# juanmc2005/diart

Hardware: AMD Instinct MI355X
Metric: real-time-factor xRT streams/GPU @500ms step (higher is better)
Workload: dtype f16x3

## Files before the change

### diart_amd/_lib.py

```python
from __future__ import annotations

import ctypes as C
import os
from pathlib import Path
from typing import Optional

EXPERIMENTS = os.environ.get("DZ_EXPERIMENTS", "0") not in ("", "0")
_LIB_PATH = Path(__file__).resolve().parent / ("libdiart_amd_exp.so" if EXPERIMENTS else "libdiart_amd.so")
_lib: Optional[C.CDLL] = None

c_float_p = C.POINTER(C.c_float)
c_double_p = C.POINTER(C.c_double)
c_int_p = C.POINTER(C.c_int)
vp = C.c_void_p


class SincNetWeights(C.Structure):
    _fields_ = [("wav_gamma", C.c_float), ("wav_beta", C.c_float)] + [
        (n, vp) for n in ("filt", "in0_g", "in0_b", "w1", "b1", "in1_g", "in1_b",
                          "w2", "b2", "in2_g", "in2_b", "w1_split", "w2_split", "filt_split")]


class SegWeights(C.Structure):
    _fields_ = [("sinc", SincNetWeights), ("wih", vp * 4), ("bih", vp * 4), ("whh", vp * 4),
# ... 92 lines not shown
    "dz_resample_out_len": (C.c_longlong, [C.c_int, C.c_int, C.c_longlong]),
    "dz_resample_table": (C.c_int, [C.c_int, C.c_int, c_float_p]),
    "dz_resample_create": (C.c_int, [vp, C.c_int, C.c_int, C.POINTER(vp)]),
    "dz_resample_forward": (C.c_int, [vp, vp, C.c_longlong, C.c_longlong, C.c_int, vp, C.c_longlong, vp]),
    "dz_resample_destroy": (C.c_int, [vp]),
    "dz_prof_enable": (C.c_int, [C.c_int]),
    "dz_prof_pause": (C.c_int, [C.c_int]),
    "dz_prof_collect": (C.c_int, []),
    "dz_prof_get": (C.c_int, [C.c_int, C.POINTER(C.c_char_p), C.POINTER(C.c_double),
                              C.POINTER(C.c_longlong), C.POINTER(C.c_longlong)]),
    "dz_osp": (C.c_int, [vp, vp, C.c_int, C.c_int, C.c_int, C.c_float, C.c_float, C.c_int,
                         C.c_int, vp, vp]),
    "dz_l2_normalize": (C.c_int, [vp, vp, C.c_int, C.c_int, C.c_float, vp]),
    "dz_results_to_host": (C.c_int, [vp, vp, vp, C.c_longlong, vp, vp, C.c_longlong, vp]),
    "dz_cdist_cosine": (C.c_int, [vp, vp, vp, C.c_int, C.c_int, C.c_int, C.c_int, vp, vp]),
    "dz_clu_create": (C.c_int, [C.c_double, C.c_double, C.c_double, C.c_int, C.POINTER(vp)]),
    "dz_clu_reset": (C.c_int, [vp]),
    "dz_clu_step": (C.c_int, [vp, vp, C.c_int, C.c_int, vp, C.c_int, vp, vp]),
    "dz_clu_step_batch": (C.c_int, [C.POINTER(vp), C.c_int, vp, C.c_int, C.c_int, vp, C.c_int,
                                    vp, vp, C.c_int]),
    "dz_clu_get_centers": (C.c_int, [vp, vp, C.c_int]),
    "dz_clu_get_active": (C.c_int, [vp, vp]),
    "dz_clu_dim": (C.c_int, [vp]),
    "dz_clu_set_state": (C.c_int, [vp, vp, vp, C.c_int]),
    "dz_clu_destroy": (C.c_int, [vp]),
    "dz_lsap": (C.c_int, [vp, C.c_int, C.c_int, vp]),
    "dz_ring_create": (C.c_int, [vp, C.c_int, C.c_int, C.c_int, C.c_int, C.POINTER(vp)]),
    "dz_ring_reset": (C.c_int, [vp]),
    "dz_ring_destroy": (C.c_int, [vp]),
    "dz_ring_push": (C.c_int, [vp, vp, C.c_longlong, C.c_int, vp]),
    "dz_ring_window": (C.c_int, [vp, C.POINTER(vp), C.POINTER(C.c_longlong), C.POINTER(C.c_int)]),
    "dz_ring_read": (C.c_int, [vp, vp, vp]),
    "dz_ring_push_rows": (C.c_int, [vp, vp, C.c_longlong, C.c_int, C.POINTER(C.c_int), C.c_int, vp]),
    "dz_ring_push_rows_pcm": (C.c_int, [vp, vp, C.c_longlong, C.c_int, C.c_int, C.c_int, C.POINTER(C.c_int), C.c_int, vp]),
    "dz_ring_filled_row": (C.c_int, [vp, C.c_int, C.POINTER(C.c_int)]),
    "dz_ring_gather": (C.c_int, [vp, C.POINTER(C.c_int), C.c_int, vp, C.c_longlong, vp]),
    "dz_ring_reset_row": (C.c_int, [vp, C.c_int]),
    "dz_tail_create": (C.c_int, [C.c_int, C.c_int, C.c_double, C.c_double, C.c_double, C.c_int,
                                 C.c_int, vp, C.POINTER(vp)]),
    "dz_tail_reset": (C.c_int, [vp]),
    "dz_tail_destroy": (C.c_int, [vp]),
    "dz_tail_max_rows": (C.c_int, [vp]),
    "dz_tail_step": (C.c_int, [vp, vp, C.c_double, C.c_double, vp, vp, vp, vp, vp, C.c_int, vp]),
    "dz_tail_step_batch": (C.c_int, [C.POINTER(vp), C.c_int, vp, vp, vp, vp, vp, vp, vp, vp,
                                     C.c_int, vp, C.c_int]),
    "dz_file_step_batch": (C.c_int, [C.POINTER(vp), C.POINTER(vp), C.c_int, vp, vp, vp, C.c_int, C.c_int, vp, C.c_int,
                                     C.c_int, vp, C.c_double, vp, C.c_int, vp, vp, C.c_int]),
    "dz_k_convgemm": (C.c_int, [vp, vp, vp]),
    "dz_k_gemm_f32": (C.c_int, [vp, vp, vp]),
    "dz_k_gemm_split": (C.c_int, [vp, vp, vp]),
    "dz_k_gemm_pre": (C.c_int, [vp, vp, vp]),
    "dz_k_mlp_head": (C.c_int, [vp, vp, C.c_longlong, vp, vp, vp, vp, vp, vp, C.c_int, C.c_int, C.c_int, C.c_int,
                                C.c_int, C.c_float, C.c_float, vp, vp, vp]),
    "dz_k_seg_head": (C.c_int, [vp, vp, vp, vp, C.c_int, C.c_int, C.c_int, C.c_int, C.c_int, vp, C.c_float,
                                C.c_float, C.c_int, vp, vp]),
    "dz_k_conv_pool": (C.c_int, [vp, vp, vp]),
    "dz_k_convgemm_ntile": (C.c_int, [C.c_int]),
    "dz_k_wave_stats": (C.c_int, [vp, vp, C.c_longlong, C.c_int, C.c_int, vp, vp]),
    "dz_k_sinc_conv0": (C.c_int, [vp, vp, C.c_longlong, C.c_int, C.c_int, vp, C.c_float,
                                  C.c_float, vp, vp, vp, vp]),
    "dz_k_sinc_conv0_split": (C.c_int, [vp, vp, C.c_longlong, C.c_int, C.c_int, vp, C.c_float,
                                        C.c_float, vp, vp, vp, vp]),
    "dz_k_conv0_split_ntile": (C.c_int, [C.c_int]),
    "dz_k_finalize_norm": (C.c_int, [vp, vp, C.c_int, C.c_int, C.c_int, C.c_int, vp, vp, vp, vp, vp]),
    "dz_k_lstm": (C.c_int, [vp, vp, vp, vp, C.c_int, C.c_int, vp]),
    "dz_k_lstm_mfma": (C.c_int, [vp, vp, vp, vp, C.c_int, C.c_int, C.c_int, C.c_int, vp]),
    "dz_k_lstm_planes": (C.c_int, [vp, vp, vp, vp, C.c_int, vp, C.c_longlong, C.c_int, C.c_int, vp]),
    "dz_k_stats_pool": (C.c_int, [vp, vp, C.c_int, C.c_int, C.c_int, vp, C.c_int, C.c_int,
                                  C.c_int, vp, C.c_int, vp]),
    "dz_k_powerset": (C.c_int, [vp, vp, C.c_int, C.c_int, C.c_int, vp, vp]),
    "dz_k_conv2d": (C.c_int, [vp, vp, vp, vp, vp, vp, vp, C.c_int, C.c_int, C.c_int, C.c_int, C.c_int, C.c_int,
                              C.c_int, C.c_int, vp]),
}


EXPERIMENT_SIGNATURES = {
    "dz_k_gemm_g2": (C.c_int, [vp, vp, C.c_int, vp]),
    "dz_k_gemm_g3": (C.c_int, [vp, vp, C.c_int, vp]),
    "dz_k_conv_pool_debug": (C.c_int, [vp]),
    "dz_sinc_conv0_pair": (C.c_int, [vp, vp, vp, C.c_longlong, C.c_int, vp, vp, vp, vp]),
    "dz_k_sinc_conv0_pair": (C.c_int, [vp, vp, C.c_longlong, C.c_int, C.c_int, vp, vp, vp, C.c_float, C.c_float, vp, vp,
                                       vp, vp, vp]),
}


class ConvGemmDesc(C.Structure):
    _fields_ = [(n, vp) for n in ("X", "W", "bias", "e0", "e1", "nscale", "nshift", "Y", "partials")] + [
        (n, C.c_int) for n in ("B", "Tin", "Tout", "Cin", "taps", "dil", "K", "Kpad", "Npad",
                               "Nstore", "ldx", "ldy", "nld", "Tstore")] + [
        ("xbs", C.c_longlong), ("ybs", C.c_longlong), ("norm_on_load", C.c_int), ("epi", C.c_int),
        ("ksplit", C.c_int), ("ysplit", C.c_longlong), ("agroup", C.c_int), ("pad", C.c_int),
        ("X2", vp), ("rowbias", vp), ("Wsplit", vp), ("Xsplit", vp), ("xplane", C.c_longlong),
        ("Ysplit", vp), ("yplane", C.c_longlong), ("npart", vp), ("ngamma", vp), ("nbeta", vp),
        ("npart_tiles", C.c_int), ("npart_T", C.c_int), ("oflag", vp), ("Tdev", vp)]


(EPI_BIAS, EPI_BIAS_LEAKY, EPI_BIAS_SIGMOID, EPI_TDNN, EPI_POOL3, EPI_BIAS_RELU, EPI_RELU_BN,
 EPI_RELU_BN_TANH) = range(8)


class DiartAmdError(RuntimeError):
    pass


def lib_path() -> Path:
    return _LIB_PATH
# ... 88 lines not shown
```

### diart_amd/csrc/api.hip

```cpp
#include "dz_common.h"

#include <stdarg.h>
#include <stdio.h>
#include <stdlib.h>
#include <string.h>
#include <mutex>
#include <new>

static thread_local char g_err[512] = "";
void dz_set_error(const char* fmt, ...) {
    va_list ap;
    va_start(ap, fmt);
    vsnprintf(g_err, sizeof(g_err), fmt, ap);
    va_end(ap);
}
extern "C" const char* dz_last_error(void) { return g_err; }
extern "C" int dz_version(void) { return DZ_VERSION; }
extern "C" int dz_abi_struct_sizes(int out[5]) {
    if (!out) return 2;
    out[0] = (int)sizeof(dz_sincnet_weights);
    out[1] = (int)sizeof(dz_seg_weights);
    out[2] = (int)sizeof(dz_emb_weights);
    out[3] = (int)sizeof(dz_ecapa_weights);
    out[4] = (int)sizeof(dz_convgemm_desc);
// ... 916 lines not shown
    DZ_REQUIRE(ctx && d, "dz_k_gemm_split: NULL argument");
    DZ_HIP(hipSetDevice(ctx->device));
    DzRangeScope range_scope(ctx->oflag_dev);
    return dz_launch_gemm_split(*d, (hipStream_t)stream);
}
extern "C" int dz_k_gemm_pre(dz_ctx* ctx, const dz_convgemm_desc* d, void* stream) {
    DZ_REQUIRE(ctx && d, "dz_k_gemm_pre: NULL argument");
    DZ_HIP(hipSetDevice(ctx->device));
    DzRangeScope range_scope(ctx->oflag_dev);
    return dz_launch_gemm_pre(*d, (hipStream_t)stream);
}
#ifdef DZ_EXPERIMENTS
extern "C" int dz_k_gemm_g2(dz_ctx* ctx, const dz_convgemm_desc* d, int row_fragments, void* stream) {
    DZ_REQUIRE(ctx && d, "dz_k_gemm_g2: NULL argument");
    DZ_REQUIRE(d->Wsplit && d->Xsplit && (d->Y || d->Ysplit) && d->B == 1 && d->K == d->Kpad && d->K == d->taps * d->Cin &&
                   d->Cin % 32 == 0 && d->Npad % 128 == 0 && d->pad == 0 && !d->X2 && !d->rowbias && d->ksplit <= 1 &&
                   !d->norm_on_load && d->Tout > 0 && d->Tout == d->Tin - (d->taps - 1) * d->dil && d->ldx % 32 == 0 &&
                   d->xplane % d->ldx == 0 && d->xplane / d->ldx >= d->Tin,
               "dz_k_gemm_g2: the requirements of dz_k_gemm_pre apply");
    DZ_HIP(hipSetDevice(ctx->device));
    DzRangeScope range_scope(ctx->oflag_dev);
    DzConvGemm p = *d;
    if (!p.oflag) p.oflag = ctx->oflag_dev;
    return dz_launch_gemm_g2(p, row_fragments, (hipStream_t)stream);
}
extern "C" int dz_k_gemm_g3(dz_ctx* ctx, const dz_convgemm_desc* d, int row_fragments, void* stream) {
    DZ_REQUIRE(ctx && d, "dz_k_gemm_g3: NULL argument");
    DZ_REQUIRE(d->Wsplit && d->Xsplit && (d->Y || d->Ysplit) && d->B == 1 && d->K == d->Kpad && d->K == d->taps * d->Cin &&
                   d->Cin % 32 == 0 && d->Npad % 128 == 0 && d->pad == 0 && !d->X2 && !d->rowbias && d->ksplit <= 1 &&
                   !d->norm_on_load && d->Tout > 0 && d->Tout == d->Tin - (d->taps - 1) * d->dil && d->ldx % 32 == 0 &&
                   d->xplane % d->ldx == 0 && d->xplane / d->ldx >= d->Tin,
               "dz_k_gemm_g3: the requirements of dz_k_gemm_pre apply");
    DZ_HIP(hipSetDevice(ctx->device));
    DzRangeScope range_scope(ctx->oflag_dev);
    DzConvGemm p = *d;
    if (!p.oflag) p.oflag = ctx->oflag_dev;
    return dz_launch_gemm_g3(p, row_fragments, (hipStream_t)stream);
}
#endif
extern "C" int dz_k_mlp_head(dz_ctx* ctx, const void* xsplit, long long xplane, const void* w0split,
                             const void* w1split, const float* b0, const float* b1, const float* cw,
                             const float* cb, int rows, int frames, int classes, int speakers, int powerset,
                             float gamma, float beta, float* d_seg, float* d_weights, void* stream) {
    DZ_REQUIRE(ctx, "dz_k_mlp_head: NULL argument");
    DZ_HIP(hipSetDevice(ctx->device));
    DzRangeScope range_scope(ctx->oflag_dev);
    DzMlpHead m{};
    m.Xsplit = xsplit; m.xplane = xplane; m.W0split = w0split; m.W1split = w1split;
    m.b0 = b0; m.b1 = b1; m.cw = cw; m.cb = cb;
    m.rows = rows; m.F = frames; m.classes = classes; m.K = speakers; m.powerset = powerset;
    m.gamma = gamma; m.beta = beta; m.seg = d_seg; m.wout = d_weights;
    return dz_launch_mlp_head(m, (hipStream_t)stream);
}
extern "C" int dz_k_seg_head(dz_ctx* ctx, const float* m1, const float* cw, const float* cb, int batch,
                             int frames, int classes, int speakers, int powerset, float* d_seg, float gamma,
                             float beta, int normalize, float* d_weights, void* stream) {
    DZ_REQUIRE(ctx && m1 && cw && cb && d_seg, "dz_k_seg_head: NULL argument");
    DZ_HIP(hipSetDevice(ctx->device));
    return dz_launch_seg_head(m1, cw, cb, batch, frames, classes, speakers, powerset, d_seg, gamma, beta,
                              normalize, d_weights, (hipStream_t)stream);
}
extern "C" int dz_k_conv_pool(dz_ctx* ctx, const dz_convgemm_desc* d, void* stream) {
    DZ_REQUIRE(ctx && d, "dz_k_conv_pool: NULL argument");
    DZ_HIP(hipSetDevice(ctx->device));
    DzRangeScope range_scope(ctx->oflag_dev);
    DZ_REQUIRE(d->Wsplit && (d->Cin == 80 || d->Cin == 64), "dz_k_conv_pool: Wsplit is NULL or Cin is not 80 / 64");
    std::lock_guard<std::mutex> frag_lock(ctx->frag_mu);
    if (!ctx->convp_frag) DZ_HIP(hipMalloc(&ctx->convp_frag, (size_t)dz_conv_pool_wfrag_bytes(80)));
    if (ctx->convp_used && ctx->convp_user != (hipStream_t)stream) DZ_HIP(hipStreamSynchronize(ctx->convp_user));
    ctx->convp_user = (hipStream_t)stream; ctx->convp_used = true;
    int rc;
    if (!(dz_option(DZ_OPT_PACK_CACHE) && ctx->convp_src == d->Wsplit && ctx->convp_cin == d->Cin && ctx->convp_kpad == d->Kpad)) {
        if ((rc = dz_launch_conv_pool_wfrag(d->Cin, d->Wsplit, d->Kpad, ctx->convp_frag, (hipStream_t)stream))) return rc;
        ctx->convp_src = d->Wsplit; ctx->convp_cin = d->Cin; ctx->convp_kpad = d->Kpad;
    }
    return dz_launch_conv_pool(*d, (hipStream_t)stream, ctx->convp_frag);
}
#ifdef DZ_EXPERIMENTS
extern "C" int dz_k_conv_pool_debug(long long* d_stamps) {
    dz_conv_pool_dbg = d_stamps;
    return 0;
}
#endif
extern "C" int dz_k_convgemm_ntile(int t_out) { return dz_convgemm_ntile(t_out); }
extern "C" int dz_k_wave_stats(dz_ctx* ctx, const float* d_wave, long long stride, int batch,
                               int samples, float* d_stats, void* stream) {
    DZ_REQUIRE(ctx && d_stats, "dz_k_wave_stats: NULL argument");
    int rc;
    if ((rc = check_wave("dz_k_wave_stats", d_wave, stride, samples))) return rc;
    DZ_HIP(hipSetDevice(ctx->device));
    float* mom = nullptr;
    DZ_HIP(hipMalloc((void**)&mom, (size_t)batch * 2 * DZ_WS_G * sizeof(float)));
    rc = dz_launch_wave_stats(d_wave, stride, batch, samples, mom, (hipStream_t)stream);
    if (!rc) rc = dz_launch_wave_stats_combine(mom, batch, samples, d_stats, (hipStream_t)stream);
    (void)hipStreamSynchronize((hipStream_t)stream);
    (void)hipFree(mom);
    return rc;
}
extern "C" int dz_k_sinc_conv0(dz_ctx* ctx, const float* d_wave, long long stride, int batch,
                               int samples, const float* d_stats, float gamma, float beta,
                               const float* d_filt, float* d_y0, float* d_partials, void* stream) {
    DZ_REQUIRE(ctx && d_stats && d_filt && d_y0 && d_partials, "dz_k_sinc_conv0: NULL argument");
    int rc;
    if ((rc = check_wave("dz_k_sinc_conv0", d_wave, stride, samples))) return rc;
    const SincGeom g = sinc_geom(samples);
    DZ_REQUIRE(g.P0 > 0, "dz_k_sinc_conv0: %d samples is too short", samples);
// ... 99 lines not shown
```

### diart_amd/csrc/dz_common.h

```cpp
#pragma once
#include <hip/hip_runtime.h>
#include <hip/hip_ext.h>
#include <stdint.h>
#include <stddef.h>
#include <mutex>
#include "../../include/diart_amd.h"

#ifdef DZ_EXPERIMENTS
#include <stdlib.h>
static inline const char* dz_exp_env(const char* name) { return getenv(name); }
#else
#define dz_exp_env(name) ((const char*)nullptr)
#endif
enum { DZ_OPT_F32_GEMM = 0, DZ_OPT_POOL_FUSE, DZ_OPT_PACK_CACHE, DZ_OPT_COUNT };
int dz_option(int id);

typedef float f32x4 __attribute__((ext_vector_type(4)));
typedef float f32x2 __attribute__((ext_vector_type(2)));

#define DZ_MFMA(a, b, c) __builtin_amdgcn_mfma_f32_16x16x4f32((a), (b), (c), 0, 0, 0)

#define DZ_LEAKY_SLOPE 0.01f

struct DzAttrOnce {
// ... 329 lines not shown
        } else if (best > K) {
            int idx = best - K - 1;
            for (int i = 0; i < K && a < 0; ++i) {
                const int cnt = K - 1 - i;
                if (idx < cnt) {
                    a = i;
                    b2 = i + 1 + idx;
                } else {
                    idx -= cnt;
                }
            }
        }
        for (int k = 0; k < K; ++k) s[k] = (k == a || k == b2) ? 1.f : 0.f;
    } else {
        for (int k = 0; k < K; ++k) s[k] = 1.f / (1.f + expf(-lg[k]));
    }
}
__device__ __forceinline__ float dz_vad_frame(const float* s, int K) {
    float m = s[0];
    for (int k = 1; k < K; ++k) m = (s[k] > m || s[k] != s[k]) ? s[k] : m;
    return m;
}
__device__ __forceinline__ void dz_osp_frame(const float* s, int K, float gamma, float beta, float* w) {
    float e[8], m = -INFINITY;
    for (int k = 0; k < K; ++k) m = fmaxf(m, beta * s[k]);
    float sum = 0.f;
    for (int k = 0; k < K; ++k) {
        e[k] = expf(beta * s[k] - m);
        sum += e[k];
    }
    for (int k = 0; k < K; ++k) {
        const float pr = e[k] / sum;
        float wv = dz_powg(s[k], gamma) * dz_powg(pr, gamma);
        if (wv < 1e-8f) wv = 1e-8f;
        w[k] = wv;
    }
}

int dz_launch_seg_head(const float* m1, const float* cw, const float* cb, int B, int F, int classes, int K,
                       int powerset, float* seg, float gamma, float beta, int normalize, float* wout,
                       hipStream_t st, const float* wave_mom = nullptr, float* vad = nullptr);
struct DzMlpHead {
    const void* Xsplit;
    long long xplane;
    const void *W0split, *W1split;
    const float *b0, *b1, *cw, *cb;
    int rows, F, classes, K, powerset;
    float gamma, beta;
    float* seg;
    float* wout;
    int* oflag;
    const float* wave_mom;
    float* vad;
};
int dz_launch_mlp_head(const DzMlpHead& p, hipStream_t st);
int dz_launch_l2norm(float* x, int rows, int dim, float norm, hipStream_t st);
int dz_launch_splitk_finish(const float* parts, int nsplit, long long stride, int rows, int dim,
                            int normalize, float* out, hipStream_t st, const float* wave_mom = nullptr,
                            int rows_per_x = 1);
int dz_launch_powerset(const float* logp, int rows, int classes, int speakers, float* out,
                       hipStream_t st);
int dz_launch_cdist(const float* emb, const double* centers, int n, int k, int g, int dim,
                    double* out, hipStream_t st);

int dz_launch_mask_compact(const float* wave, long long stride, int S, const float* masks, int Fw,
                           int rows, float* sig, long long sig_stride, int* lens, hipStream_t st,
                           int rows_per_wave = 1);
int dz_launch_ecapa_geometry(const int* lens, int G, int K, int Tc, int min_samples, int hop, int* nvalid,
                             int* nmask, int* tooshort, int* tdev, int* rv, int* rm, int* rt, hipStream_t st);
int dz_launch_power(const float* spec, int lds, long long rows, float* pw, hipStream_t st);
int dz_launch_fbank_post(const float* melp, int T, int rows, const int* nvalid, float* feats,
                         hipStream_t st, const int* tdev = nullptr);
int dz_launch_se_mean(const float* x, int T, int C, int ldx, int rows, const int* nmask, float* s,
                      hipStream_t st);
int dz_launch_se_apply(const float* x, int ldx, const float* gate, const float* resid, int ldr,
                       float* out, int ldo, int rows, int T, int C, hipStream_t st);
int dz_launch_se_apply_planes(const float* x, int ldx, const float* gate, const float* resid, int ldr, float* out,
                              int ldo, void* planes, long long plane, int rows, int T, int C, hipStream_t st);
int dz_launch_asp_gstats(const float* x, int T, int C, int rows, const int* nmask, float* g,
                         hipStream_t st);
int dz_launch_asp_pool(const float* x, const float* logit, int T, int C, int rows, const int* nmask,
                       float* pooled, hipStream_t st);
int dz_launch_nan_rows(float* out, int rows, int dim, const int* flags, hipStream_t st);
int dz_launch_fbank_post_mels(const float* melp, int n_mels, int T, int rows, const int* nvalid, float* feats,
                              hipStream_t st, const int* tdev = nullptr);
int dz_launch_sb_stats_pool(const float* x, int T, int C, int ldx, int rows, const int* nvalid, float mean_bias,
                            float std_bias, float* pooled, hipStream_t st);

struct DzConv2d {
    const float* X;
    const float* W;
    const void* Wsplit;
    const float* bias;
    const float* R;
    float* Y;
    int B, Fi, Ti, Cin, Fo, To, Cout, taps, stride, relu;
    int* oflag;
};
int dz_launch_conv2d(const DzConv2d& p, hipStream_t st);

int dz_launch_wsp_fbank(const float* wave, long long stride, int N, int T, const float* mel, float* raw, int* bad,
                        hipStream_t st);
int dz_launch_wsp_cmn(const float* raw, int N, int T, const int* bad, float* feats, hipStream_t st);
int dz_launch_wsp_conv1(const float* feats, int N, int T, const float* w, const float* b, float* y, hipStream_t st);
int dz_launch_wsp_pool(const float* x, int B, int T4, const float* weights, int Fw, int K, const int* bad,
                       float* out, int* rflag, hipStream_t st);
// ... 19 lines not shown
```

### diart_amd/csrc/k_mlp_head.hip

```cpp
#include "dz_common.h"

namespace {

typedef _Float16 f16x8 __attribute__((ext_vector_type(8)));
typedef _Float16 f16x4 __attribute__((ext_vector_type(4)));
typedef float f32x16 __attribute__((ext_vector_type(16)));

constexpr int PLANE = 128 * 64;
constexpr int R0 = 0, R1 = 8 * PLANE;
constexpr int M1_PITCH = 129;
constexpr int PAR = R1 + 128 * M1_PITCH * 4 + 64;
constexpr int PAR_B0 = 0, PAR_B1 = 128, PAR_CW = 256, PAR_CB = 256 + 8 * 128;
constexpr size_t LDS_BYTES = PAR + (PAR_CB + 8) * sizeof(float);
constexpr float LO_UNSCALE = 1.f / 2048.f;

__device__ __forceinline__ float leaky(float v) { return v > 0.f ? v : v * DZ_LEAKY_SLOPE; }

__global__ __launch_bounds__(256) void mlp_head_kernel(DzMlpHead p) {
    extern __shared__ __attribute__((aligned(16))) char smem[];
    const int tid = threadIdx.x;
    const int w = __builtin_amdgcn_readfirstlane(tid >> 6), l = tid & 63;
    const int t0 = blockIdx.x * 128;

    float* par = reinterpret_cast<float*>(smem + PAR);
    if (tid < 128) {
        par[PAR_B0 + tid] = p.b0[tid];
        par[PAR_B1 + tid] = p.b1[tid];
    }
    for (int i = tid; i < p.classes * 128; i += 256) par[PAR_CW + i] = p.cw[i];
    if (tid < p.classes) par[PAR_CB + tid] = p.cb[tid];

    const bool isB = w >= 2;
    const int lo = w & 1;
    const unsigned short* A = reinterpret_cast<const unsigned short*>(p.Xsplit);
    const unsigned short* W0 = reinterpret_cast<const unsigned short*>(p.W0split);
    const unsigned short* W1 = reinterpret_cast<const unsigned short*>(p.W1split);
    const unsigned short* src = isB ? W0 + (long long)lo * 128 * 256 : A + (long long)lo * p.xplane;
    const unsigned nbytes = (unsigned)((isB ? 128ll : (long long)p.rows) * 256 * 2);
    const __amdgpu_buffer_rsrc_t rsrc = __builtin_amdgcn_make_buffer_rsrc((void*)src, 0, nbytes, 0x00020000);
    const int chunk = ((l & 3) ^ ((l >> 4) & 3)) << 4;
    const int voff0 = ((isB ? 0 : t0) + (l >> 2)) * 64 + chunk;
    const int kb_bytes = (isB ? 128 : p.rows) * 64;
    auto issue0 = [&](int kt, int stage) {
        char* dst = smem + R0 + stage * 4 * PLANE + w * PLANE;
#pragma unroll
        for (int i = 0; i < 8; ++i)
            __builtin_amdgcn_raw_ptr_buffer_load_lds(
                rsrc, (__attribute__((address_space(3))) void*)(dst + i * 1024), 16, voff0 + i * 1024, kt * kb_bytes, 0, 0);
    };
    const __amdgpu_buffer_rsrc_t rs1 = __builtin_amdgcn_make_buffer_rsrc((void*)W1, 0, 2u * 128 * 128 * 2, 0x00020000);
    auto issue1 = [&]() {
        const int voff1 = (l >> 2) * 64 + chunk;
#pragma unroll
        for (int pl = 0; pl < 2; ++pl)
#pragma unroll
            for (int i = 0; i < 8; ++i)
                __builtin_amdgcn_raw_ptr_buffer_load_lds(
                    rs1, (__attribute__((address_space(3))) void*)(smem + R0 + w * 2 * PLANE + pl * PLANE + i * 1024), 16,
                    voff1 + i * 1024 + pl * (128 * 128 * 2), w * (128 * 64), 0, 0);
    };

    const int li = l & 31, g = l >> 5;
    const int wm = w >> 1, wn = w & 1;
    const int sw = (li >> 2) & 3;
    int foff[2];
#pragma unroll
    for (int ks = 0; ks < 2; ++ks) foff[ks] = li * 64 + (((2 * ks + g) ^ sw) << 4);
    f32x16 accm[2][2], accx[2][2];
    auto zero = [&]() {
#pragma unroll
        for (int mt = 0; mt < 2; ++mt)
#pragma unroll
// ... 62 lines not shown
    }
    dz_flag_range(p.oflag, amax);

    zero();
    asm volatile("s_waitcnt vmcnt(0) lgkmcnt(0)\n\ts_barrier" ::: "memory");
#pragma unroll
    for (int kt = 0; kt < 4; ++kt) compute(smem + R1 + kt * 2 * PLANE, smem + R0 + kt * 2 * PLANE);
    asm volatile("s_waitcnt lgkmcnt(0)\n\ts_barrier" ::: "memory");

    float* m1 = reinterpret_cast<float*>(smem + R1);
#pragma unroll
    for (int mt = 0; mt < 2; ++mt) {
        const int row = wm * 64 + mt * 32 + li;
#pragma unroll
        for (int nt = 0; nt < 2; ++nt)
#pragma unroll
            for (int k = 0; k < 4; ++k) {
                const int n = wn * 64 + nt * 32 + 8 * k + 4 * g;
                const f32x4 bv = *reinterpret_cast<const f32x4*>(par + PAR_B1 + n);
#pragma unroll
                for (int e = 0; e < 4; ++e)
                    m1[row * M1_PITCH + n + e] =
                        leaky((accm[mt][nt][4 * k + e] + accx[mt][nt][4 * k + e] * LO_UNSCALE) + bv[e]);
            }
    }
    __syncthreads();

    const int t = t0 + tid;
    if (tid < 128 && t < p.rows) {
        const float* x = m1 + tid * M1_PITCH;
        float lg[8];
        for (int c = 0; c < p.classes; ++c) {
            float acc = 0.f;
            const float* wc = par + PAR_CW + c * 128;
#pragma unroll 8
            for (int k = 0; k < 128; ++k) acc = fmaf(x[k], wc[k], acc);
            lg[c] = acc + par[PAR_CB + c];
        }
        float s[8];
        dz_seg_decide(lg, p.classes, p.K, p.powerset, s);
        const int b = t / p.F, f = t - b * p.F;
        if (p.wave_mom && dz_ws_bad(p.wave_mom, b))
            for (int k = 0; k < p.K; ++k) s[k] = __builtin_nanf("");
        for (int k = 0; k < p.K; ++k) p.seg[(long long)t * p.K + k] = s[k];
        if (p.vad) p.vad[t] = dz_vad_frame(s, p.K);
        if (p.wout) {
            float wv[8];
            dz_osp_frame(s, p.K, p.gamma, p.beta, wv);
            for (int k = 0; k < p.K; ++k) p.wout[((long long)b * p.K + k) * p.F + f] = wv[k];
        }
    }
}

}

int dz_launch_mlp_head(const DzMlpHead& p_in, hipStream_t st) {
    DzMlpHead p = p_in;
    if (!p.oflag) p.oflag = dz_cur_oflag;
    DZ_REQUIRE(p.Xsplit && p.W0split && p.W1split && p.b0 && p.b1 && p.cw && p.cb && p.seg, "mlp_head: NULL argument");
    DZ_REQUIRE(p.rows > 0 && p.F > 0 && p.rows % p.F == 0, "mlp_head: %d rows are not whole chunks of %d frames", p.rows, p.F);
    DZ_REQUIRE(p.classes >= 1 && p.classes <= 8 && p.K >= 1 && p.K <= 8 && (p.powerset || p.K == p.classes),
               "mlp_head: classes %d / speakers %d", p.classes, p.K);
    DZ_REQUIRE((long long)p.rows * 256 * 2 < (1ll << 31), "mlp_head: plane exceeds the buffer range");
    DZ_REQUIRE(p.xplane == (long long)p.rows * 256, "mlp_head: kb-major input planes of exactly `rows` rows (xplane = rows * 256)");
    static DzAttrOnce attr_once;
    DZ_HIP(attr_once.raise((const void*)mlp_head_kernel, (int)LDS_BYTES));
    DZ_LAUNCH(mlp_head_kernel, dim3((p.rows + 127) / 128), dim3(256), LDS_BYTES, st, p);
    DZ_HIP(hipGetLastError());
    return 0;
}
```

### include/diart_amd.h

```cpp
#ifndef DIART_AMD_H
#define DIART_AMD_H

#ifdef __cplusplus
extern "C" {
#endif

#define DZ_VERSION 230

typedef struct dz_ctx dz_ctx;
typedef struct dz_seg dz_seg;
typedef struct dz_emb dz_emb;
typedef struct dz_clu dz_clu;

const char* dz_last_error(void);
int dz_version(void);
int dz_set_option(const char* name, int value);
int dz_get_option(const char* name, int* value);
int dz_has_experiments(void);
int dz_host_pool_set_spin(int microseconds);

int dz_ctx_create(int hip_device, dz_ctx** out);
int dz_ctx_destroy(dz_ctx* ctx);
int dz_range_check(dz_ctx* ctx, int reset);

// ... 187 lines not shown
           float* d_out, void* stream);

int dz_results_to_host(dz_ctx* ctx, const float* d_a, float* h_a, long long n_a,
                       const float* d_b, float* h_b, long long n_b, void* stream);

int dz_l2_normalize(dz_ctx* ctx, float* d_emb, int rows, int dim, float norm, void* stream);

int dz_cdist_cosine(dz_ctx* ctx, const float* d_emb, const double* d_centers,
                    int n_streams, int k_local, int g_global, int dim,
                    double* d_out, void* stream);

enum { DZ_EPI_BIAS = 0, DZ_EPI_BIAS_LEAKY = 1, DZ_EPI_BIAS_SIGMOID = 2, DZ_EPI_TDNN = 3,
       DZ_EPI_POOL3 = 4, DZ_EPI_BIAS_RELU = 5, DZ_EPI_RELU_BN = 6, DZ_EPI_RELU_BN_TANH = 7 };
typedef struct {
    const float* X;
    const float* W;
    const float* bias;
    const float* e0;
    const float* e1;
    const float* nscale;
    const float* nshift;
    float* Y;
    float* partials;
    int B, Tin, Tout, Cin, taps, dil, K, Kpad, Npad, Nstore, ldx, ldy, nld, Tstore;
    long long xbs, ybs;
    int norm_on_load;
    int epi;
    int ksplit;
    long long ysplit;
    int agroup;
    int pad;
    const float* X2;
    const float* rowbias;
    const void* Wsplit;
    const void* Xsplit;
    long long xplane;
    void* Ysplit;
    long long yplane;
    const float* npart;
    const float* ngamma;
    const float* nbeta;
    int npart_tiles, npart_T;
    int* oflag;
    const int* Tdev;
} dz_convgemm_desc;
int dz_k_convgemm(dz_ctx* ctx, const dz_convgemm_desc* desc, void* stream);
int dz_k_gemm_f32(dz_ctx* ctx, const dz_convgemm_desc* desc, void* stream);
int dz_k_gemm_split(dz_ctx* ctx, const dz_convgemm_desc* desc, void* stream);
int dz_k_gemm_pre(dz_ctx* ctx, const dz_convgemm_desc* desc, void* stream);
int dz_k_mlp_head(dz_ctx* ctx, const void* xsplit, long long xplane, const void* w0split, const void* w1split,
                  const float* b0, const float* b1, const float* cw, const float* cb, int rows, int frames,
                  int classes, int speakers, int powerset, float gamma, float beta, float* d_seg,
                  float* d_weights, void* stream);
int dz_k_seg_head(dz_ctx* ctx, const float* m1, const float* cw, const float* cb, int batch, int frames,
                  int classes, int speakers, int powerset, float* d_seg, float gamma, float beta,
                  int normalize, float* d_weights, void* stream);
int dz_k_conv_pool(dz_ctx* ctx, const dz_convgemm_desc* desc, void* stream);
int dz_k_convgemm_ntile(int t_out);
int dz_k_wave_stats(dz_ctx* ctx, const float* d_wave, long long stride, int batch, int samples,
                    float* d_stats, void* stream);
int dz_k_sinc_conv0(dz_ctx* ctx, const float* d_wave, long long stride, int batch, int samples,
                    const float* d_stats, float gamma, float beta, const float* d_filt,
                    float* d_y0, float* d_partials, void* stream);
int dz_k_sinc_conv0_split(dz_ctx* ctx, const float* d_wave, long long stride, int batch, int samples,
                          const float* d_stats, float gamma, float beta, const void* d_filt_split,
                          float* d_y0, float* d_partials, void* stream);
int dz_k_conv0_split_ntile(int samples);
int dz_k_finalize_norm(dz_ctx* ctx, const float* d_partials, int batch, int ntile, int channels,
                       int frames, const float* d_gamma, const float* d_beta, float* d_scale,
                       float* d_shift, void* stream);
int dz_k_lstm(dz_ctx* ctx, const float* d_gx, const float* d_whh, float* d_hout, int batch,
              int frames, void* stream);
int dz_k_lstm_mfma(dz_ctx* ctx, const float* d_gx, const void* d_whh_split, float* d_hout,
                   int batch, int frames, int unit_major, int variant, void* stream);
int dz_k_lstm_planes(dz_ctx* ctx, const float* d_gx, const float* d_whh, const void* d_whh_split,
                     int variant, void* d_hsplit, long long hplane, int batch, int frames, void* stream);
int dz_k_stats_pool(dz_ctx* ctx, const float* d_x, int frames, int channels, int ldx,
                    const float* d_weights, int weight_frames, int rows, int rows_per_x,
                    float* d_out, int ldo, void* stream);
int dz_k_powerset(dz_ctx* ctx, const float* d_logits, int rows, int classes, int speakers,
                  float* d_out, void* stream);

int dz_clu_create(double tau_active, double rho_update, double delta_new,
                  int max_speakers, dz_clu** out);
int dz_clu_reset(dz_clu* clu);
int dz_clu_step(dz_clu* clu, const float* seg, int frames, int k_local,
                const float* emb, int dim, double* scores_out, int* assign_out);
int dz_clu_step_batch(dz_clu** clus, int n, const float* seg, int frames, int k_local,
                      const float* emb, int dim, double* scores_out, int* assign_out,
                      int num_threads);
int dz_clu_get_centers(dz_clu* clu, double* out, int dim);
int dz_clu_get_active(dz_clu* clu, int* out_mask);
int dz_clu_dim(dz_clu* clu);
int dz_clu_set_state(dz_clu* clu, const double* centers, const int* active_mask, int dim);
int dz_clu_destroy(dz_clu* clu);

int dz_prof_enable(int on);
int dz_prof_pause(int paused);
int dz_prof_collect(void);
int dz_prof_get(int tag, const char** name, double* total_ms, long long* launches,
                long long* chunks);

typedef struct dz_ring dz_ring;
int dz_ring_create(dz_ctx* ctx, int n_streams, int window, int hop, int slack_blocks, dz_ring** out);
int dz_ring_reset(dz_ring* r);
int dz_ring_destroy(dz_ring* r);
// ... 44 lines not shown
```

Before: 33190.

## Add a 64-row tile variant of the MLP head kernel and make it default

```diff
diff --git a/diart_amd/_lib.py b/diart_amd/_lib.py
--- a/diart_amd/_lib.py
+++ b/diart_amd/_lib.py
@@ -168,6 +168,8 @@
     "dz_k_gemm_pre": (C.c_int, [vp, vp, vp]),
     "dz_k_mlp_head": (C.c_int, [vp, vp, C.c_longlong, vp, vp, vp, vp, vp, vp, C.c_int, C.c_int, C.c_int, C.c_int,
                                 C.c_int, C.c_float, C.c_float, vp, vp, vp]),
+    "dz_k_mlp_head_form": (C.c_int, [vp, vp, C.c_longlong, vp, vp, vp, vp, vp, vp, C.c_int, C.c_int, C.c_int, C.c_int,
+                                     C.c_int, C.c_float, C.c_float, vp, vp, vp, vp, C.c_int, vp]),
     "dz_k_seg_head": (C.c_int, [vp, vp, vp, vp, C.c_int, C.c_int, C.c_int, C.c_int, C.c_int, vp, C.c_float,
                                 C.c_float, C.c_int, vp, vp]),
     "dz_k_conv_pool": (C.c_int, [vp, vp, vp]),
diff --git a/diart_amd/csrc/api.hip b/diart_amd/csrc/api.hip
--- a/diart_amd/csrc/api.hip
+++ b/diart_amd/csrc/api.hip
@@ -992,6 +992,22 @@
     m.gamma = gamma; m.beta = beta; m.seg = d_seg; m.wout = d_weights;
     return dz_launch_mlp_head(m, (hipStream_t)stream);
 }
+extern "C" int dz_k_mlp_head_form(dz_ctx* ctx, const void* xsplit, long long xplane, const void* w0split,
+                                  const void* w1split, const float* b0, const float* b1, const float* cw,
+                                  const float* cb, int rows, int frames, int classes, int speakers, int powerset,
+                                  float gamma, float beta, float* d_seg, float* d_weights, float* d_vad,
+                                  const float* d_wave_stats, int form, void* stream) {
+    DZ_REQUIRE(ctx, "dz_k_mlp_head_form: NULL argument");
+    DZ_HIP(hipSetDevice(ctx->device));
+    DzRangeScope range_scope(ctx->oflag_dev);
+    DzMlpHead m{};
+    m.Xsplit = xsplit; m.xplane = xplane; m.W0split = w0split; m.W1split = w1split;
+    m.b0 = b0; m.b1 = b1; m.cw = cw; m.cb = cb;
+    m.rows = rows; m.F = frames; m.classes = classes; m.K = speakers; m.powerset = powerset;
+    m.gamma = gamma; m.beta = beta; m.seg = d_seg; m.wout = d_weights; m.vad = d_vad; m.wave_mom = d_wave_stats;
+    m.form = form;
+    return dz_launch_mlp_head(m, (hipStream_t)stream);
+}
 extern "C" int dz_k_seg_head(dz_ctx* ctx, const float* m1, const float* cw, const float* cb, int batch,
                              int frames, int classes, int speakers, int powerset, float* d_seg, float gamma,
                              float beta, int normalize, float* d_weights, void* stream) {
diff --git a/diart_amd/csrc/dz_common.h b/diart_amd/csrc/dz_common.h
--- a/diart_amd/csrc/dz_common.h
+++ b/diart_amd/csrc/dz_common.h
@@ -405,6 +405,7 @@
     int* oflag;
     const float* wave_mom;
     float* vad;
+    int form;
 };
 int dz_launch_mlp_head(const DzMlpHead& p, hipStream_t st);
 int dz_launch_l2norm(float* x, int rows, int dim, float norm, hipStream_t st);
diff --git a/diart_amd/csrc/k_mlp_head.hip b/diart_amd/csrc/k_mlp_head.hip
--- a/diart_amd/csrc/k_mlp_head.hip
+++ b/diart_amd/csrc/k_mlp_head.hip
@@ -16,8 +16,7 @@
 
 __device__ __forceinline__ float leaky(float v) { return v > 0.f ? v : v * DZ_LEAKY_SLOPE; }
 
-__global__ __launch_bounds__(256) void mlp_head_kernel(DzMlpHead p) {
-    extern __shared__ __attribute__((aligned(16))) char smem[];
+__device__ __forceinline__ void mlp_head_rows128(const DzMlpHead& p, char* smem) {
     const int tid = threadIdx.x;
     const int w = __builtin_amdgcn_readfirstlane(tid >> 6), l = tid & 63;
     const int t0 = blockIdx.x * 128;
@@ -186,6 +185,225 @@
     }
 }
 
+template <int MT>
+struct Small {
+    static constexpr int ROWS = 32 * MT;
+    static constexpr int APLANE = ROWS * 64;
+    static constexpr int STAGE = 2 * APLANE + 2 * PLANE;
+    static constexpr int L1A = 0, M1 = 8 * APLANE;
+    static constexpr int LG = 0;
+    static constexpr int PAR = 3 * STAGE > M1 + ROWS * M1_PITCH * 4 ? 3 * STAGE : M1 + ROWS * M1_PITCH * 4;
+    static constexpr size_t LDS_BYTES = PAR + (PAR_CB + 8) * sizeof(float);
+    static_assert(PAR % 16 == 0, "parameter block alignment");
+};
+static_assert(2 * Small<2>::LDS_BYTES <= 160 * 1024, "two workgroups of the 64-row form per CU");
+
+template <int MT>
+__device__ __forceinline__ void mlp_head_small(const DzMlpHead& p, char* smem) {
+    typedef Small<MT> S;
+    constexpr int APLANE = S::APLANE;
+    const int tid = threadIdx.x;
+    const int w = __builtin_amdgcn_readfirstlane(tid >> 6), l = tid & 63;
+    const int t0 = blockIdx.x * S::ROWS;
+    const int li = l & 31, g = l >> 5;
+    const int sw = (li >> 2) & 3;
+
+    f16x8 b1h[4][2], b1l[4][2];
+    {
+        const char* W1 = reinterpret_cast<const char*>(p.W1split) + (w * 32 + li) * 64 + (g << 4);
+#pragma unroll
+        for (int kt = 0; kt < 4; ++kt)
+#pragma unroll
+            for (int ks = 0; ks < 2; ++ks) {
+                b1h[kt][ks] = *reinterpret_cast<const f16x8*>(W1 + kt * (128 * 64) + ks * 32);
+                b1l[kt][ks] = *reinterpret_cast<const f16x8*>(W1 + 128 * 128 * 2 + kt * (128 * 64) + ks * 32);
+            }
+    }
+
+    const bool isB = w >= 2;
+    const int lo = w & 1;
+    const unsigned short* A = reinterpret_cast<const unsigned short*>(p.Xsplit);
+    const unsigned short* W0 = reinterpret_cast<const unsigned short*>(p.W0split);
+    const unsigned short* src = isB ? W0 + (long long)lo * 128 * 256 : A + (long long)lo * p.xplane;
+    const unsigned nbytes = (unsigned)((isB ? 128ll : (long long)p.rows) * 256 * 2);
+    const __amdgpu_buffer_rsrc_t rsrc = __builtin_amdgcn_make_buffer_rsrc((void*)src, 0, nbytes, 0x00020000);
+    const int chunk = ((l & 3) ^ ((l >> 4) & 3)) << 4;
+    const int voff0 = ((isB ? 0 : t0) + (l >> 2)) * 64 + chunk;
+    const int kb_bytes = (isB ? 128 : p.rows) * 64;
+    const int plane_off = isB ? 2 * APLANE + lo * PLANE : lo * APLANE;
+    auto issue0 = [&](int kt, int stage) {
+        char* dst = smem + stage * S::STAGE + plane_off;
+#pragma unroll
+        for (int i = 0; i < 2 * MT; ++i)
+            __builtin_amdgcn_raw_ptr_buffer_load_lds(
+                rsrc, (__attribute__((address_space(3))) void*)(dst + i * 1024), 16, voff0 + i * 1024, kt * kb_bytes, 0, 0);
+        if (isB) {
+#pragma unroll
+            for (int i = 2 * MT; i < 8; ++i)
+                __builtin_amdgcn_raw_ptr_buffer_load_lds(
+                    rsrc, (__attribute__((address_space(3))) void*)(dst + i * 1024), 16, voff0 + i * 1024, kt * kb_bytes, 0, 0);
+        }
+    };
+    auto wait_stage = [&](bool more) {
+        if (!more) asm volatile("s_waitcnt vmcnt(0) lgkmcnt(0)\n\ts_barrier" ::: "memory");
+        else if (isB) asm volatile("s_waitcnt vmcnt(8) lgkmcnt(0)\n\ts_barrier" ::: "memory");
+        else asm volatile("s_waitcnt vmcnt(%0) lgkmcnt(0)\n\ts_barrier" ::"n"(2 * MT) : "memory");
+    };
+
+    int foff[2];
+#pragma unroll
+    for (int ks = 0; ks < 2; ++ks) foff[ks] = li * 64 + (((2 * ks + g) ^ sw) << 4);
+    f32x16 accm[MT], accx[MT];
+    auto zero = [&]() {
+#pragma unroll
+        for (int mt = 0; mt < MT; ++mt)
+#pragma unroll
+            for (int r = 0; r < 16; ++r) accm[mt][r] = accx[mt][r] = 0.f;
+    };
+    auto mfma3 = [&](const f16x8 (&ah)[MT], const f16x8 (&al)[MT], const f16x8& bh, const f16x8& bl) {
+#pragma unroll
+        for (int mt = 0; mt < MT; ++mt) {
+            accx[mt] = __builtin_amdgcn_mfma_f32_32x32x16_f16(bh, al[mt], accx[mt], 0, 0, 0);
+            accm[mt] = __builtin_amdgcn_mfma_f32_32x32x16_f16(bh, ah[mt], accm[mt], 0, 0, 0);
+            accx[mt] = __builtin_amdgcn_mfma_f32_32x32x16_f16(bl, ah[mt], accx[mt], 0, 0, 0);
+        }
+    };
+    auto load_a = [&](const char* a_hi, int ks, f16x8 (&ah)[MT], f16x8 (&al)[MT]) {
+#pragma unroll
+        for (int t = 0; t < MT; ++t) {
+            ah[t] = *reinterpret_cast<const f16x8*>(a_hi + t * 2048 + foff[ks]);
+            al[t] = *reinterpret_cast<const f16x8*>(a_hi + APLANE + t * 2048 + foff[ks]);
+        }
+    };
+
+    zero();
+    issue0(0, 0);
+    issue0(1, 1);
+    float* par = reinterpret_cast<float*>(smem + S::PAR);
+    if (tid < 128) {
+        par[PAR_B0 + tid] = p.b0[tid];
+        par[PAR_B1 + tid] = p.b1[tid];
+    }
+    for (int i = tid; i < p.classes * 128; i += 256) par[PAR_CW + i] = p.cw[i];
+    if (tid < p.classes) par[PAR_CB + tid] = p.cb[tid];
+#pragma unroll
+    for (int kt = 0; kt < 8; ++kt) {
+        wait_stage(kt + 1 < 8);
+        if (kt + 2 < 8) issue0(kt + 2, (kt + 2) % 3);
+        const char* st = smem + (kt % 3) * S::STAGE;
+        const char* sb = st + 2 * APLANE + (w * 32) * 64;
+#pragma unroll
+        for (int ks = 0; ks < 2; ++ks) {
+            f16x8 ah[MT], al[MT];
+            load_a(st, ks, ah, al);
+            const f16x8 bh = *reinterpret_cast<const f16x8*>(sb + foff[ks]);
+            const f16x8 bl = *reinterpret_cast<const f16x8*>(sb + PLANE + foff[ks]);
+            mfma3(ah, al, bh, bl);
+        }
+    }
+    asm volatile("s_waitcnt lgkmcnt(0)\n\ts_barrier" ::: "memory");
+
+    float amax = 0.f;
+#pragma unroll
+    for (int mt = 0; mt < MT; ++mt) {
+        const int row = mt * 32 + li;
+#pragma unroll
+        for (int k = 0; k < 4; ++k) {
+            const int n = w * 32 + 8 * k + 4 * g;
+            const f32x4 bv = *reinterpret_cast<const f32x4*>(par + PAR_B0 + n);
+            f32x4 v;
+#pragma unroll
+            for (int e = 0; e < 4; ++e) {
+                float x = leaky((accm[mt][4 * k + e] + accx[mt][4 * k + e] * LO_UNSCALE) + bv[e]);
+                amax = fmaxf(amax, fabsf(x));
+                v[e] = __builtin_amdgcn_fmed3f(x, -65504.f, 65504.f);
+            }
+            const f16x4 hi = __builtin_convertvector(v, f16x4);
+            const f16x4 lo4 = __builtin_convertvector((v - __builtin_convertvector(hi, f32x4)) * 2048.f, f16x4);
+            char* d = smem + S::L1A + w * 2 * APLANE + row * 64 + ((k ^ ((row >> 2) & 3)) << 4) + 8 * g;
+            *reinterpret_cast<f16x4*>(d) = hi;
+            *reinterpret_cast<f16x4*>(d + APLANE) = lo4;
+        }
+    }
+    dz_flag_range(p.oflag, amax);
+
+    zero();
+    asm volatile("s_waitcnt vmcnt(0) lgkmcnt(0)\n\ts_barrier" ::: "memory");
+#pragma unroll
+    for (int kt = 0; kt < 4; ++kt)
+#pragma unroll
+        for (int ks = 0; ks < 2; ++ks) {
+            f16x8 ah[MT], al[MT];
+            load_a(smem + S::L1A + kt * 2 * APLANE, ks, ah, al);
+            mfma3(ah, al, b1h[kt][ks], b1l[kt][ks]);
+        }
+
+    float* m1 = reinterpret_cast<float*>(smem + S::M1);
+#pragma unroll
+    for (int mt = 0; mt < MT; ++mt) {
+        const int row = mt * 32 + li;
+#pragma unroll
+        for (int k = 0; k < 4; ++k) {
+            const int n = w * 32 + 8 * k + 4 * g;
+            const f32x4 bv = *reinterpret_cast<const f32x4*>(par + PAR_B1 + n);
+#pragma unroll
+            for (int e = 0; e < 4; ++e)
+                m1[row * M1_PITCH + n + e] = leaky((accm[mt][4 * k + e] + accx[mt][4 * k + e] * LO_UNSCALE) + bv[e]);
+        }
+    }
+    __syncthreads();
+
+    float* lgs = reinterpret_cast<float*>(smem + S::LG);
+    if (w < p.classes) {
+        const bool two = w + 4 < p.classes;
+        const float* wc0 = par + PAR_CW + w * 128;
+        const float* wc1 = par + PAR_CW + (two ? w + 4 : w) * 128;
+        for (int row = l; row < S::ROWS; row += 64) {
+            const float* x = m1 + row * M1_PITCH;
+            float acc0 = 0.f, acc1 = 0.f;
+#pragma unroll 8
+            for (int k = 0; k < 128; ++k) {
+                const float xv = x[k];
+                acc0 = fmaf(xv, wc0[k], acc0);
+                acc1 = fmaf(xv, wc1[k], acc1);
+            }
+            lgs[row * 8 + w] = acc0 + par[PAR_CB + w];
+            if (two) lgs[row * 8 + w + 4] = acc1 + par[PAR_CB + w + 4];
+        }
+    }
+    __syncthreads();
+
+    const int t = t0 + tid;
+    if (tid < S::ROWS && t < p.rows) {
+        float lg[8];
+        for (int c = 0; c < p.classes; ++c) lg[c] = lgs[tid * 8 + c];
+        float s[8];
+        dz_seg_decide(lg, p.classes, p.K, p.powerset, s);
+        const int b = t / p.F, f = t - b * p.F;
+        if (p.wave_mom && dz_ws_bad(p.wave_mom, b))
+            for (int k = 0; k < p.K; ++k) s[k] = __builtin_nanf("");
+        for (int k = 0; k < p.K; ++k) p.seg[(long long)t * p.K + k] = s[k];
+        if (p.vad) p.vad[t] = dz_vad_frame(s, p.K);
+        if (p.wout) {
+            float wv[8];
+            dz_osp_frame(s, p.K, p.gamma, p.beta, wv);
+            for (int k = 0; k < p.K; ++k) p.wout[((long long)b * p.K + k) * p.F + f] = wv[k];
+        }
+    }
+}
+
+__global__ __launch_bounds__(256) void mlp_head_kernel(DzMlpHead p) {
+    extern __shared__ __attribute__((aligned(16))) char smem[];
+    mlp_head_rows128(p, smem);
+}
+
+namespace rows64 {
+__global__ __launch_bounds__(256, 2) void mlp_head_kernel(DzMlpHead p) {
+    extern __shared__ __attribute__((aligned(16))) char smem[];
+    mlp_head_small<2>(p, smem);
+}
+}
+
 }
 
 int dz_launch_mlp_head(const DzMlpHead& p_in, hipStream_t st) {
@@ -197,9 +415,16 @@
                "mlp_head: classes %d / speakers %d", p.classes, p.K);
     DZ_REQUIRE((long long)p.rows * 256 * 2 < (1ll << 31), "mlp_head: plane exceeds the buffer range");
     DZ_REQUIRE(p.xplane == (long long)p.rows * 256, "mlp_head: kb-major input planes of exactly `rows` rows (xplane = rows * 256)");
-    static DzAttrOnce attr_once;
-    DZ_HIP(attr_once.raise((const void*)mlp_head_kernel, (int)LDS_BYTES));
-    DZ_LAUNCH(mlp_head_kernel, dim3((p.rows + 127) / 128), dim3(256), LDS_BYTES, st, p);
+    DZ_REQUIRE(p.form == 0 || p.form == 64 || p.form == 128, "mlp_head: form %d (0, 64 or 128)", p.form);
+    if (p.form == 0) p.form = 64;
+    static DzAttrOnce attr_once, attr_once64;
+    if (p.form == 64) {
+        DZ_HIP(attr_once64.raise((const void*)rows64::mlp_head_kernel, (int)Small<2>::LDS_BYTES));
+        DZ_LAUNCH(rows64::mlp_head_kernel, dim3((p.rows + 63) / 64), dim3(256), Small<2>::LDS_BYTES, st, p);
+    } else {
+        DZ_HIP(attr_once.raise((const void*)mlp_head_kernel, (int)LDS_BYTES));
+        DZ_LAUNCH(mlp_head_kernel, dim3((p.rows + 127) / 128), dim3(256), LDS_BYTES, st, p);
+    }
     DZ_HIP(hipGetLastError());
     return 0;
 }
diff --git a/include/diart_amd.h b/include/diart_amd.h
--- a/include/diart_amd.h
+++ b/include/diart_amd.h
@@ -263,6 +263,10 @@
                   const float* b0, const float* b1, const float* cw, const float* cb, int rows, int frames,
                   int classes, int speakers, int powerset, float gamma, float beta, float* d_seg,
                   float* d_weights, void* stream);
+int dz_k_mlp_head_form(dz_ctx* ctx, const void* xsplit, long long xplane, const void* w0split, const void* w1split,
+                       const float* b0, const float* b1, const float* cw, const float* cb, int rows, int frames,
+                       int classes, int speakers, int powerset, float gamma, float beta, float* d_seg,
+                       float* d_weights, float* d_vad, const float* d_wave_stats, int form, void* stream);
 int dz_k_seg_head(dz_ctx* ctx, const float* m1, const float* cw, const float* cb, int batch, int frames,
                   int classes, int speakers, int powerset, float* d_seg, float gamma, float beta,
                   int normalize, float* d_weights, void* stream);
```

Result: no change. 32910 (-0.8%).
